# cc-ai/climategan

Hardware: AMD Instinct MI355X
Metric: 640x640 images/sec (G+D step): per-domain sample slots per second of the joint Masker+Painter training step (update_G + update_D), global batch 32 per domain (higher is better)
Workload: dtype bf16

## Files before the change

### climategan_amd/_lib.py

```python
import ctypes as C
import os
from pathlib import Path

_HERE = Path(__file__).resolve().parent
LIB_PATH = Path(os.environ["CGAN_LIB"]).resolve() if os.environ.get("CGAN_LIB") else _HERE / "libcgan_hip.so"

CGAN_F16, CGAN_BF16, CGAN_F32 = 0, 1, 2
ACT_NONE, ACT_RELU, ACT_LRELU, ACT_TANH, ACT_SIGMOID = 0, 1, 2, 3, 4
PAD_ZERO, PAD_REFLECT = 0, 1
ABI_VERSION = 1


class ConvDesc(C.Structure):
    _fields_ = [
        ("dtype", C.c_int32), ("n", C.c_int32), ("h_in", C.c_int32), ("w_in", C.c_int32),
        ("c_in", C.c_int32), ("c_out", C.c_int32),
        ("kh", C.c_int32), ("kw", C.c_int32), ("stride", C.c_int32), ("pad", C.c_int32), ("dilation", C.c_int32),
        ("pad_mode", C.c_int32), ("h_out", C.c_int32), ("w_out", C.c_int32), ("in_upsample", C.c_int32),
        ("act", C.c_int32), ("act_slope", C.c_float), ("has_bias", C.c_int32), ("has_residual", C.c_int32),
        ("residual_upsample", C.c_int32),
    ]


class NormStatsDesc(C.Structure):
# ... 121 lines not shown
    "cgan_spade_packed_weight_bytes": (C.c_size_t, [C.POINTER(SpadeDesc)]),
    "cgan_spade_pack_weights": (C.c_int, [_P, _P, _P, _P, _P, _P, _P, C.POINTER(SpadeDesc), _P]),
    "cgan_spade_fused_fwd": (C.c_int, [_P, _P, _P, _P, _P, _P, C.POINTER(SpadeDesc), _P]),
    "cgan_spade_fused_fwd_train": (C.c_int, [_P, _P, _P, _P, _P, _P, _P, C.POINTER(SpadeDesc), _P]),
    "cgan_spectral_norm_workspace_bytes": (C.c_size_t, [C.c_int32, C.c_int32]),
    "cgan_spectral_norm_power_iter": (C.c_int, [_P, _P, _P, _P, C.c_int32, C.c_int32, _P, C.c_size_t, _P]),
    "cgan_spectral_norm_power_iter_batched": (C.c_int, [_P, C.c_int32, C.c_int32, C.c_int32, _P]),
    "cgan_extra_adam_multi_tensor": (C.c_int, [_P, C.c_int32, C.c_int64, C.c_int32, C.c_int32, C.c_int32, C.c_double,
                                               C.c_double, C.c_double, C.c_double, C.c_double, _P]),
    "cgan_grads_nonfinite_check_multi_tensor": (C.c_int, [_P, C.c_int32, C.c_int64, C.c_double, C.c_int32, _P, _P]),
    "cgan_adam_multi_tensor": (C.c_int, [_P, C.c_int32, C.c_int64] + [C.c_double] * 6 + [_P, _P]),
    "cgan_rmsprop_multi_tensor": (C.c_int, [_P, C.c_int32, C.c_int64] + [C.c_double] * 5 + [_P, _P]),
    "cgan_amp_optim_finish": (C.c_int, [_P, C.c_int32, _P, _P]),
    "cgan_nchw_to_nhwc": (C.c_int, [_P, _P, _P, C.c_int32, C.c_int32, C.c_int32, C.c_int32, C.c_int32, C.c_int32, _P]),
    "cgan_nhwc_to_nchw": (C.c_int, [_P, _P, _P, _P, C.c_int32, C.c_int32, C.c_int32, C.c_int32, C.c_int32, C.c_int32, _P]),
    "cgan_resize_nearest_nhwc": (C.c_int, [_P, _P, C.c_int32, C.c_int32, C.c_int32, C.c_int32, C.c_int32, C.c_int32,
                                           C.c_int32, C.c_int32, C.c_int32, _P]),
    "cgan_avgpool3x3s2_nhwc": (C.c_int, [_P, _P, C.c_int32, C.c_int32, C.c_int32, C.c_int32, C.c_int32, _P]),
    "cgan_maxpool3x3s2_nhwc": (C.c_int, [_P, _P, C.c_int32, C.c_int32, C.c_int32, C.c_int32, C.c_int32, _P]),
    "cgan_resize_bilinear_nhwc": (C.c_int, [_P, _P, C.c_int32, C.c_int32, C.c_int32, C.c_int32, C.c_int32, C.c_int32,
                                            C.c_int32, C.c_int32, _P]),
    "cgan_resize_bicubic_nhwc": (C.c_int, [_P, _P, C.c_int32, C.c_int32, C.c_int32, C.c_int32, C.c_int32, C.c_int32,
                                           C.c_int32, _P]),
    "cgan_sumpool2x2_nhwc": (C.c_int, [_P, _P, C.c_int32, C.c_int32, C.c_int32, C.c_int32, C.c_int32, _P]),
    "cgan_reflect_pad_bwd_nhwc": (C.c_int, [_P, _P, C.c_int32, C.c_int32, C.c_int32, C.c_int32, C.c_int32, C.c_int32, _P]),
    "cgan_copy_channels_nhwc": (C.c_int, [_P, _P, C.c_int64, C.c_int32, C.c_int32, C.c_int32, C.c_int32, _P]),
    "cgan_eltwise_nhwc": (C.c_int, [_P, _P, _P, C.c_int32, C.c_int32, C.c_int64, _P]),
    "cgan_fold_bn": (C.c_int, [_P, _P, _P, _P, _P, _P, C.c_float, _P, _P, C.c_int32, C.c_int64, _P]),
    "cgan_act_bwd": (C.c_int, [_P, _P, _P, C.c_int32, C.c_int32, C.c_float, C.c_int64, _P]),
    "cgan_instnorm_act_bwd_workspace_bytes": (C.c_size_t, [C.POINTER(NormStatsDesc)]),
    "cgan_instnorm_act_bwd": (C.c_int, [_P, _P, _P, _P, C.POINTER(NormStatsDesc), C.c_int32, C.c_float, _P, C.c_size_t,
                                        _P]),
    "cgan_spade_bwd_prepare": (C.c_int, [_P, _P, _P, _P, _P, _P, _P, _P, _P, C.POINTER(SpadeDesc), _P]),
    "cgan_spade_hidden_bwd_workspace_bytes": (C.c_size_t, [C.POINTER(SpadeDesc)]),
    "cgan_spade_hidden_bwd": (C.c_int, [_P, _P, _P, _P, _P, _P, _P, _P, C.c_size_t, C.POINTER(SpadeDesc), _P]),
    "cgan_batchnorm_train_stats": (C.c_int, [_P, _P, _P, C.c_float, _P, _P, _P, _P, _P, _P, _P, C.POINTER(NormStatsDesc), _P,
                                             C.c_size_t, _P]),
    "cgan_batchnorm_train_stats_from_partials": (C.c_int, [_P, C.c_int32, _P, _P, C.c_float, _P, _P, _P, _P, _P, _P, _P,
                                                           C.POINTER(NormStatsDesc), _P]),
    "cgan_conv2d_stats_chunk_pixels": (C.c_int32, [C.POINTER(ConvDesc)]),
    "cgan_conv2d_nhwc_fwd_stats": (C.c_int, [_P, _P, _P, _P, _P, C.c_size_t, C.POINTER(ConvDesc), _P]),
    "cgan_bn_train_prepare": (C.c_int, [_P, _P, _P, _P, C.c_float, C.c_float, C.c_int64, _P, _P, _P, _P, _P, C.c_int32, _P]),
    "cgan_batchnorm_act_bwd_workspace_bytes": (C.c_size_t, [C.c_int32]),
    "cgan_batchnorm_act_bwd": (C.c_int, [_P, _P, _P, _P, _P, _P, _P, _P, _P, _P, _P, _P, C.c_int32, C.c_int64, C.c_int32,
                                         C.c_int32, C.c_float, _P, C.c_size_t, _P]),
    "cgan_batchnorm_act_bwd_grouped": (C.c_int, [_P, _P, _P, _P, _P, _P, _P, _P, _P, _P, _P, _P, C.c_int32, C.c_int64,
                                                 C.c_int32, C.c_int32, C.c_int32, C.c_float, _P, C.c_size_t, _P]),
    "cgan_bce_logits_nhwc": (C.c_int, [_P, C.c_int32, C.c_int64, C.c_int32, C.c_float, C.c_float, _P, _P, _P]),
    "cgan_hinge_nhwc": (C.c_int, [_P, C.c_int32, C.c_int64, C.c_int32, C.c_int32, C.c_int32, C.c_float, _P, _P, _P]),
    "cgan_l1_nhwc": (C.c_int, [_P, _P, C.c_int32, C.c_int64, C.c_float, _P, _P, _P]),
    "cgan_mse_const_nhwc": (C.c_int, [_P, C.c_int32, C.c_int64, C.c_int32, C.c_float, C.c_float, _P, _P, _P]),
    "cgan_painter_aux_losses": (C.c_int, [_P, _P, _P, C.c_int32, C.c_int32, C.c_int32, C.c_int32, C.c_float, C.c_float,
                                          C.c_float, C.c_float, _P, _P, _P]),
    "cgan_resize_bicubic_bwd_nhwc": (C.c_int, [_P, _P, C.c_int32, C.c_int32, C.c_int32, C.c_int32, C.c_int32, C.c_int32,
                                               C.c_int32, _P]),
    "cgan_spectral_norm_bwd": (C.c_int, [_P, _P, _P, _P, _P, C.c_int32, C.c_int32, _P, _P]),
    "cgan_painter_heads_fwd": (C.c_int, [_P, _P, _P, _P, _P, C.c_int32, C.c_int32, C.c_int32, C.c_int32, _P]),
    "cgan_painter_heads_bwd": (C.c_int, [_P, _P, _P, _P, C.c_int32, C.c_int32, C.c_int32, C.c_int32, _P]),
    "cgan_diffaug_fwd": (C.c_int, [_P, _P, _P, _P, C.c_int32, C.c_int32, C.c_int32, C.c_int32, C.c_int32, C.c_int32,
                                   C.c_int32, _P, _P]),
    "cgan_diffaug_bwd": (C.c_int, [_P, _P, _P, _P, C.c_int32, C.c_int32, C.c_int32, C.c_int32, C.c_int32, C.c_int32,
                                   C.c_int32, _P, _P]),
    "cgan_painter_heads_diffaug_fwd": (C.c_int, [_P, _P, _P, _P, _P, _P, _P, C.c_int32, C.c_int32, C.c_int32, C.c_int32,
                                                 C.c_int32, C.c_int32, C.c_int32, _P, _P]),
    "cgan_painter_heads_diffaug_bwd": (C.c_int, [_P, _P, _P, _P, _P, _P, C.c_int32, C.c_int32, C.c_int32, C.c_int32,
                                                 C.c_int32, C.c_int32, C.c_int32, _P, _P]),
# ... 149 lines not shown
```

### climategan_amd/autograd.py

```python
import ctypes as C

import os

import torch

from . import ops


GRAD_SCALE = 1.0


def set_grad_scale(s: float):
    global GRAD_SCALE
    GRAD_SCALE = float(s)


BN_GROUPS = 1


class bn_groups:

    def __init__(self, groups: int):
        self.groups = int(groups)

# ... 197 lines not shown
                                       pad_mode=cfg.get("pad_mode", ops.PAD_ZERO), add=add, prepacked=ctx.dgrad,
                                       relu_out=relu_out).t
        dw = db = None
        if ctx.needs_input_grad[1] or (ctx.has_bias and ctx.needs_input_grad[2]):
            dw, db = ops.conv2d_bwd_weight(
                ops.NHWC(x_t, cfg["c_in"]), dy, tuple(weight.shape), stride=cfg["stride"], pad=cfg["pad"],
                dilation=cfg["dilation"], want_bias=ctx.has_bias, pad_mode=cfg.get("pad_mode", ops.PAD_ZERO))
        return dx_t, dw, db, None, None


class InstNormActFn(torch.autograd.Function):

    @staticmethod
    def forward(ctx, x_t, c, eps, act, slope):
        x = ops.NHWC(x_t, c)
        mean, rstd = ops.instnorm_stats(x, eps=eps)
        out = ops.norm_act_apply(x, mean, rstd, act=act, slope=slope)
        ctx.c, ctx.act, ctx.slope = c, act, slope
        ctx.save_for_backward(out.t, rstd)
        return out.t

    @staticmethod
    def backward(ctx, dy_t):
        out_t, rstd = ctx.saved_tensors
        dx = ops.instnorm_act_bwd(ops.NHWC(out_t, ctx.c), ops.NHWC(dy_t.contiguous(), ctx.c), rstd, act=ctx.act,
                                  slope=ctx.slope)
        return dx.t, None, None, None, None


_SPADE_REMAT_GAMMA = os.environ.get("CGAN_SPADE_REMAT_GAMMA") == "1"


_SPADE_FUSED_BWD = os.environ.get("CGAN_SPADE_FUSED_BWD", "1") != "0"


class SpadeFn(torch.autograd.Function):

    @staticmethod
    def forward(ctx, x_t, cond_t, mean, rstd, w_sh, b_sh, w_g, b_g, w_b, b_b, packed, cfg):
        x = ops.NHWC(x_t, cfg["c"])
        cond = ops.NHWC(cond_t, cfg["cond_c"])
        gamma_t = None
        if _SPADE_REMAT_GAMMA or not any(ctx.needs_input_grad):
            y = ops.spade_fused(x, mean, rstd, cond, packed, act=cfg["act"], slope=cfg["slope"],
                                x_upsample=cfg["x_upsample"])
        else:
            y, gamma = ops.spade_fused(x, mean, rstd, cond, packed, act=cfg["act"], slope=cfg["slope"],
                                       x_upsample=cfg["x_upsample"], want_gamma=True)
            gamma_t = gamma.t
        ctx.cfg = cfg
        ctx.save_for_backward(x_t, cond_t, mean, rstd, y.t, w_sh, b_sh, w_g, b_g, w_b, b_b, gamma_t)
        return y.t

    @staticmethod
    def backward(ctx, dy_t):
        cfg = ctx.cfg
        x_t, cond_t, mean, rstd, y_t, w_sh, b_sh, w_g, b_g, w_b, b_b, gamma_t = ctx.saved_tensors
        c, dt = cfg["c"], y_t.dtype
        x, y = ops.NHWC(x_t, c), ops.NHWC(y_t, c)
        dy = ops.NHWC(dy_t.contiguous(), c)
        h, w = y.h, y.w
        seg = ops.resize_nearest(ops.NHWC(cond_t, cfg["cond_c"]), (h, w), cs_out=ops.cs8(cfg["cond_c"]))
        pw_sh = ops.pack_conv_weight(w_sh, b_sh, dt)
        actv = ops.conv2d(seg, pw_sh, pad=1, act=ops.ACT_RELU)
        gamma = ops.NHWC(gamma_t, c) if gamma_t is not None else ops.conv2d(actv, ops.pack_conv_weight(w_g, b_g, dt), pad=1)
        dgb, xhat, dxhat = ops.spade_bwd_prepare(dy, y, x, mean, rstd, gamma, act=cfg["act"], slope=cfg["slope"],
                                                 x_upsample=cfg["x_upsample"])
        del gamma
        w_gb = torch.cat([w_g.detach(), w_b.detach()], dim=0)
        want_gb, want_sh = any(ctx.needs_input_grad[6:10]), any(ctx.needs_input_grad[4:6])
        dw_gb = db_gb = dw_sh = db_sh = None
        if want_gb:
            dw_gb, db_gb = ops.conv2d_bwd_weight(actv, dgb, tuple(w_gb.shape), pad=1)
        fused = (_SPADE_FUSED_BWD and want_sh and not ctx.needs_input_grad[1] and cfg["cond_c"] <= 4 and h * w >= 6400
                 and w_sh.shape[0] == 128 and dgb.t.nbytes < ops.ABI_MAX_BYTES and seg.t.nbytes < ops.ABI_MAX_BYTES)
        d_pre = None
        if fused:
            dw_sh, db_sh = ops.spade_hidden_bwd(dgb, w_gb, seg, pw_sh, c)
        elif want_sh or ctx.needs_input_grad[1]:
            d_pre = ops.conv2d_bwd_data(dgb, w_gb, (actv.n, h, w), pad=1, relu_out=actv)
        del dgb, actv
        if want_sh and not fused:
            dw_sh, db_sh = ops.conv2d_bwd_weight(seg, d_pre, tuple(w_sh.shape), pad=1)
        dcond_t = None
        if ctx.needs_input_grad[1]:
            d_seg = ops.conv2d_bwd_data(d_pre, w_sh.detach(), (seg.n, h, w), pad=1)
            dcond_t = ops.resize_nearest_bwd(d_seg, (cond_t.shape[1], cond_t.shape[2]), cond_t.shape[3]).t
        del d_pre
        if cfg.get("batch_stats"):
            nn_, hh, ww, cs = xhat.t.shape
            dx = ops.instnorm_act_bwd(ops.NHWC(xhat.t.view(1, nn_ * hh * ww, 1, cs), c),
                                      ops.NHWC(dxhat.t.view(1, nn_ * hh * ww, 1, cs), c), rstd[0:1].contiguous(),
                                      act=ops.ACT_NONE)
            dx = ops.NHWC(dx.t.view(nn_, hh, ww, cs), c)
        else:
            dx = ops.instnorm_act_bwd(xhat, dxhat, rstd, act=ops.ACT_NONE)
        if cfg["x_upsample"]:
            dx = ops.sumpool2x2(dx)
        dx_t = dx.t if ctx.needs_input_grad[0] else None
        if not want_gb:
            return (dx_t, dcond_t, None, None, dw_sh, db_sh, None, None, None, None, None, None)
        return (dx_t, dcond_t, None, None, dw_sh, db_sh, dw_gb[:c].contiguous(), db_gb[:c].contiguous(),
                dw_gb[c:].contiguous(), db_gb[c:].contiguous(), None, None)


class MakeMCondFn(torch.autograd.Function):

    @staticmethod
    def forward(ctx, d_t, s_t, x, s_c):
        ctx.s_c, ctx.with_x = s_c, x is not None
        ctx.save_for_backward(d_t, s_t)
        return ops.make_m_cond(ops.NHWC(d_t, 1), ops.NHWC(s_t, s_c), x).t

    @staticmethod
    def backward(ctx, dcond_t):
        d_t, s_t = ctx.saved_tensors
        cond_c = 1 + ctx.s_c + (3 if ctx.with_x else 0)
        dd, ds = ops.make_m_cond_bwd(ops.NHWC(dcond_t.contiguous(), cond_c), ops.NHWC(d_t, 1), ops.NHWC(s_t, ctx.s_c),
                                     ctx.with_x)
        return dd.t, ds.t, None, None


class PainterHeadsFn(torch.autograd.Function):

    @staticmethod
    def forward(ctx, fake_t, x, m, want_d, want_vgg):
        d_in, v_in = ops.painter_heads(ops.NHWC(fake_t, 3), x, m, fake_t.dtype, want_d, want_vgg)
        ctx.save_for_backward(m)
        ctx.want = (want_d, want_vgg)
        empty = fake_t.new_empty(0)
# ... 547 lines not shown
```

### climategan_amd/csrc/train_ops.hip

```cpp
#include "cgan_common.h"

namespace {

__host__ __device__ inline int grid_for_n(long total) {
  long g = (total + 255) / 256;
  return (int)(g < 1 ? 1 : (g > 8192 ? 8192 : g));
}

__device__ __forceinline__ float act_grad_from_out(float out, int act, float slope) {
  switch (act) {
    case CGAN_ACT_RELU: return out > 0.f ? 1.f : 0.f;
    case CGAN_ACT_LRELU: return out > 0.f ? 1.f : slope;
    case CGAN_ACT_TANH: return 1.f - out * out;
    case CGAN_ACT_SIGMOID: return out * (1.f - out);
    default: return 1.f;
  }
}

template <typename T>
__global__ void act_bwd_kernel(const uint16_t* __restrict__ out, const uint16_t* dy, uint16_t* dx, int act, float slope,
                               long groups) {
  for (long i = (long)blockIdx.x * blockDim.x + threadIdx.x; i < groups; i += (long)gridDim.x * blockDim.x) {
    const u32x4 o = CGAN_LD_STREAM(reinterpret_cast<const u32x4*>(out) + i);
    const u32x4 g = CGAN_LD_STREAM(reinterpret_cast<const u32x4*>(dy) + i);
// ... 206 lines not shown
        const float xh = live ? (xv[hh] - mean[(long)n * cs + ch]) * rstd[(long)n * cs + ch] : 0.f;
        rxh[hh] = xh;
        rdx[hh] = dz * (1.f + g2[hh]);
        rdg[hh] = dz * xh;
        dbeta[2 * e + hh] = dz;
      }
      oxh[e] = pack2<T>(rxh[0], rxh[1]);
      odx[e] = pack2<T>(rdx[0], rdx[1]);
      odg[e] = pack2<T>(rdg[0], rdg[1]);
    }
    CGAN_ST_STREAM(oxh, reinterpret_cast<u32x4*>(xhat) + i);
    CGAN_ST_STREAM(odx, reinterpret_cast<u32x4*>(dxhat) + i);
    uint16_t* row = dgb + pix * cs2;
    if (cg * 8 + 8 <= c) {
      *reinterpret_cast<u32x4*>(row + cg * 8) = odg;
    } else {
#pragma unroll
      for (int e = 0; e < 8; ++e)
        if (cg * 8 + e < c) row[cg * 8 + e] = (uint16_t)((odg[e >> 1] >> ((e & 1) * 16)) & 0xffffu);
    }
    if (cg * 8 + 8 <= c && (c & 3) == 0) {
      const u32x4 obt = {pack2<T>(dbeta[0], dbeta[1]), pack2<T>(dbeta[2], dbeta[3]), pack2<T>(dbeta[4], dbeta[5]),
                         pack2<T>(dbeta[6], dbeta[7])};
      if ((c & 7) == 0) {
        *reinterpret_cast<u32x4*>(row + c + cg * 8) = obt;
      } else {
        *reinterpret_cast<u32x2*>(row + c + cg * 8) = (u32x2){obt[0], obt[1]};
        *reinterpret_cast<u32x2*>(row + c + cg * 8 + 4) = (u32x2){obt[2], obt[3]};
      }
    } else {
#pragma unroll
      for (int e = 0; e < 8; ++e)
        if (cg * 8 + e < c) row[c + cg * 8 + e] = bits_of<T>(dbeta[e]);
    }
  }
}

__global__ void bn_train_prepare_kernel(const float* __restrict__ mean, const float* __restrict__ rstd,
                                        const float* __restrict__ gamma, const float* __restrict__ beta, float eps,
                                        float momentum, float count, float* __restrict__ running_mean,
                                        float* __restrict__ running_var, float* __restrict__ mean_out,
                                        float* __restrict__ rstd_out, long long* __restrict__ num_batches_tracked, int c,
                                        int cs) {
  const int ch = blockIdx.x * blockDim.x + threadIdx.x;
  if (ch == 0 && num_batches_tracked) *num_batches_tracked += 1;
  if (ch >= cs) return;
  float m = 0.f, r = 0.f;
  if (ch < c) {
    const float mu = mean[ch], rs = rstd[ch];
    r = rs * (gamma ? gamma[ch] : 1.f);
    m = mu - ((beta && r != 0.f) ? beta[ch] / r : 0.f);
    if (running_mean) {
      const float var_b = 1.f / (rs * rs) - eps;
      const float var_u = count > 1.f ? var_b * count / (count - 1.f) : var_b;
      running_mean[ch] = (1.f - momentum) * running_mean[ch] + momentum * mu;
      running_var[ch] = (1.f - momentum) * running_var[ch] + momentum * var_u;
    }
  }
  mean_out[ch] = m;
  rstd_out[ch] = r;
}

constexpr int BN_BWD_MAX_CHUNKS = 512;
template <int MASK>
__device__ __forceinline__ float bn_bwd_act_grad(float ov, float xv, float fm, float fr, float gneg) {
  if (MASK == 0) return 1.f;
// ... 312 lines not shown
    long blocks = (d->hw + (long)rows * 4 - 1) / ((long)rows * 4);
    const long cap = 8192 / d->n > 0 ? 8192 / d->n : 1;
    blocks = blocks < 1 ? 1 : (blocks > cap ? cap : blocks);
    DISPATCH_T(d->dtype, in_bwd_apply_kernel, dim3((unsigned)blocks, d->n), dim3(256), 0, s, (const uint16_t*)out,
               (const uint16_t*)dy, rstd, (const float*)workspace, (uint16_t*)dx, d->hw, cs, d->c, act, act_slope);
  }
  CGAN_CHECK_LAUNCH("instnorm_act_bwd");
  return CGAN_OK;
}

extern "C" int cgan_spade_bwd_prepare(const void* dy, const void* y, const void* x, const float* mean, const float* rstd,
                                      const void* gamma, void* dgb, void* xhat, void* dxhat, const CganSpadeDesc* d,
                                      void* stream) {
  CGAN_REQUIRE(d && dy && y && x && mean && rstd && gamma && dgb && xhat && dxhat, "spade_bwd_prepare: null pointer");
  CGAN_REQUIRE(d->dtype == CGAN_F16 || d->dtype == CGAN_BF16, "spade_bwd_prepare: bad dtype %d", d->dtype);
  CGAN_REQUIRE(d->n > 0 && d->h > 0 && d->w > 0 && d->c > 0, "spade_bwd_prepare: bad shape");
  CGAN_REQUIRE(d->act == CGAN_ACT_NONE || d->act == CGAN_ACT_LRELU, "spade_bwd_prepare: Unsupported activation: %d", d->act);
  if (d->x_upsample) CGAN_REQUIRE((d->h % 2) == 0 && (d->w % 2) == 0, "spade_bwd_prepare: x_upsample needs even h/w");
  const int cs = cgan_cs(d->c), cs2 = cgan_cs(2 * d->c);
  const long npix = (long)d->n * d->h * d->w;
  hipStream_t s = (hipStream_t)stream;
  if (cs2 != 2 * d->c) {
    hipError_t e = hipMemsetAsync(dgb, 0, (size_t)npix * cs2 * 2, s);
    if (e != hipSuccess) {
      cgan_set_error("spade_bwd_prepare: hipMemsetAsync failed: %s", hipGetErrorString(e));
      return CGAN_ERR_HIP;
    }
  }
  const long groups = npix * (cs / 8);
  DISPATCH_T(d->dtype, spade_bwd_prepare_kernel, dim3(grid_for_n(groups)), dim3(256), 0, s, (const uint16_t*)dy,
             (const uint16_t*)y, (const uint16_t*)x, mean, rstd, (const uint16_t*)gamma, (uint16_t*)dgb, (uint16_t*)xhat,
             (uint16_t*)dxhat, d->h, d->w, d->c, cs, cs2, d->x_upsample, d->act, d->act_slope, groups);
  CGAN_CHECK_LAUNCH("spade_bwd_prepare");
  return CGAN_OK;
}

extern "C" int cgan_bn_train_prepare(const float* batch_mean, const float* batch_rstd, const float* gamma,
                                     const float* beta, float eps, float momentum, int64_t count, float* running_mean,
                                     float* running_var, float* mean_out, float* rstd_out,
                                     int64_t* num_batches_tracked, int32_t c, void* stream) {
  CGAN_REQUIRE(batch_mean && batch_rstd && mean_out && rstd_out, "bn_train_prepare: null pointer");
  CGAN_REQUIRE((running_mean == nullptr) == (running_var == nullptr), "bn_train_prepare: running stats go together");
  CGAN_REQUIRE(c > 0 && count > 0, "bn_train_prepare: bad shape");
  const int cs = cgan_cs(c);
  hipLaunchKernelGGL(bn_train_prepare_kernel, dim3((cs + 255) / 256), dim3(256), 0, (hipStream_t)stream, batch_mean,
                     batch_rstd, gamma, beta, eps, momentum, (float)count, running_mean, running_var, mean_out, rstd_out,
                     (long long*)num_batches_tracked, c, cs);
  CGAN_CHECK_LAUNCH("bn_train_prepare");
  return CGAN_OK;
}

extern "C" size_t cgan_batchnorm_act_bwd_workspace_bytes(int32_t c) {
  return c > 0 ? (size_t)cgan_cs(c) * (3 + 2 * (size_t)BN_BWD_MAX_CHUNKS) * sizeof(float) : 0;
}

extern "C" int cgan_batchnorm_act_bwd(const void* x, const void* out, const void* dy, const float* batch_mean,
                                      const float* batch_rstd, const float* gamma, const float* fold_mean,
                                      const float* fold_rstd, void* dx, float* dgamma, float* dbeta, void* dz_out,
                                      int32_t dtype, int64_t npix, int32_t c, int32_t act, float act_slope,
                                      void* workspace, size_t workspace_bytes, void* stream) {
  return cgan_batchnorm_act_bwd_grouped(x, out, dy, batch_mean, batch_rstd, gamma, fold_mean, fold_rstd, dx, dgamma, dbeta,
                                        dz_out, dtype, npix, c, 1, act, act_slope, workspace, workspace_bytes, stream);
}

extern "C" int cgan_batchnorm_act_bwd_grouped(const void* x, const void* out, const void* dy, const float* batch_mean,
                                              const float* batch_rstd, const float* gamma, const float* fold_mean,
// ... 75 lines not shown
```

### climategan_amd/ops.py

```python
import collections
import ctypes as C
import functools
import inspect
import os
from dataclasses import dataclass
from typing import Optional, Tuple

import torch

from . import _lib
from ._lib import (ACT_LRELU, ACT_NONE, ACT_RELU, ACT_SIGMOID, ACT_TANH, CGAN_BF16, CGAN_F16, PAD_REFLECT,
                   PAD_ZERO, ConvDesc, NormStatsDesc, PackItem, SnItem, SpadeDesc)

_DT = {torch.float16: CGAN_F16, torch.bfloat16: CGAN_BF16}


def touch(*tensors) -> None:
    ts = [t for t in tensors if t is not None]
    if ts:
        torch.autograd.graph.increment_version(ts)


MAX_MAP_BYTES = 2 ** 31
ABI_MAX_BYTES = 2 ** 31
# ... 1345 lines not shown
    if x.c != pk.c or cond.c != pk.cond_c:
        raise RuntimeError("spade_fused: channel mismatch (x %d vs %d, cond %d vs %d)" % (x.c, pk.c, cond.c, pk.cond_c))
    if cond.cs != cs4(cond.c):
        raise RuntimeError("spade_fused: cond must be stored with round_up(cond_c,4) channels")
    if x.t.dtype != pk.dtype or cond.t.dtype != pk.dtype:
        raise RuntimeError("spade_fused: dtype mismatch")
    h, w = (x.h * 2, x.w * 2) if x_upsample else (x.h, x.w)
    d = _spade_desc(x.dtype_id, x.n, h, w, x.c, x_upsample, cond.h, cond.w, cond.c, act, slope)
    y = _empty((x.n, h, w, x.cs), dtype=x.t.dtype, device=x.t.device)
    lib = _lib.load()
    if want_gamma:
        gamma = _empty_like(y)
        _lib.check(lib.cgan_spade_fused_fwd_train(_ptr(x.t), _ptr(mean), _ptr(rstd), _ptr(cond.t), _ptr(pk.buf), _ptr(y),
                                                  _ptr(gamma), C.byref(d), _stream()), "cgan_spade_fused_fwd_train")
        return NHWC(y, x.c), NHWC(gamma, x.c)
    _lib.check(lib.cgan_spade_fused_fwd(_ptr(x.t), _ptr(mean), _ptr(rstd), _ptr(cond.t), _ptr(pk.buf), _ptr(y),
                                        C.byref(d), _stream()), "cgan_spade_fused_fwd")
    return NHWC(y, x.c)


@_batch_chunked("dy", "y", "x", "mean", "rstd", "gamma", out_bytes_per_sample=lambda g: g("y").h * g("y").w * cs8(2 * g("y").c) * 2)
def spade_bwd_prepare(dy: NHWC, y: NHWC, x: NHWC, mean, rstd, gamma: NHWC, act=ACT_NONE, slope=0.2, x_upsample=False):
    _need_cuda(dy.t, y.t, x.t, mean, rstd, gamma.t)
    c = y.c
    d = _spade_desc(y.dtype_id, y.n, y.h, y.w, c, x_upsample, y.h, y.w, 3, act, slope)
    dgb = _empty((y.n, y.h, y.w, cs8(2 * c)), dtype=y.t.dtype, device=y.t.device)
    xhat = _empty_like(y.t)
    dxhat = _empty_like(y.t)
    lib = _lib.load()
    _lib.check(lib.cgan_spade_bwd_prepare(_ptr(dy.t), _ptr(y.t), _ptr(x.t), _ptr(mean), _ptr(rstd), _ptr(gamma.t),
                                          _ptr(dgb), _ptr(xhat), _ptr(dxhat), C.byref(d), _stream()),
               "cgan_spade_bwd_prepare")
    return NHWC(dgb, 2 * c), NHWC(xhat, c), NHWC(dxhat, c)


@_batch_chunked("x", "mean", "rstd", "gamma", "beta")
def pair_spade_apply(x: "PairMap", mean, rstd, gamma: "PairMap", beta: "PairMap", act=ACT_NONE, slope=0.2,
                     x_upsample=False) -> "PairMap":
    _need_cuda(x.t, mean, rstd, gamma.t, beta.t)
    h, w = (x.h * 2, x.w * 2) if x_upsample else (x.h, x.w)
    if (gamma.n, gamma.h, gamma.w, gamma.c) != (x.n, h, w, x.c) or gamma.t.shape != beta.t.shape or gamma.t.dtype != x.t.dtype:
        raise RuntimeError("pair_spade_apply: gamma / beta must be pair maps of x's channels at the output extent")
    y = _empty((x.n, h, w, x.nb * x.cs), dtype=x.t.dtype, device=x.t.device)
    _lib.check(_lib.load().cgan_pair_spade_apply(_ptr(x.t), _ptr(mean), _ptr(rstd), _ptr(gamma.t), _ptr(beta.t), _ptr(y), x.dtype_id,
                                                 x.n, h, w, x.c, int(bool(x_upsample)), int(act), float(slope), _stream()),
               "cgan_pair_spade_apply")
    return PairMap(y, x.c)


def spade_hidden_bwd(dgb: NHWC, w_gb: torch.Tensor, seg: NHWC, pw_shared: PackedConv, c: int, want_bias=True):
    _need_cuda(dgb.t, w_gb, seg.t)
    n, h, w = dgb.n, dgb.h, dgb.w
    hidden = w_gb.shape[1]
    if seg.c > 4 or hidden != 128 or (seg.n, seg.h, seg.w) != (n, h, w) or dgb.c != 2 * c or w_gb.shape[0] != 2 * c:
        raise RuntimeError("spade_hidden_bwd: needs a <= 4-channel conditioning image at the map's extent and hidden width 128")
    lib = _lib.load()
    w_gb = w_gb.detach().contiguous().float()
    dconv = _conv_desc(dgb.dtype_id, n, h, w, hidden, 2 * c, 3, 3, 1, 1, 1, PAD_ZERO, has_bias=False)
    nbytes = lib.cgan_conv2d_dgrad_packed_weight_bytes(C.byref(dconv))
    if nbytes == 0:
        _lib.check(-1, "cgan_conv2d_dgrad_packed_weight_bytes")
    packed = _empty(nbytes, dtype=torch.uint8, device=w_gb.device)
    _lib.check(lib.cgan_conv2d_pack_weight_dgrad(_ptr(w_gb), _ptr(None), _ptr(packed), C.byref(dconv), _stream()),
               "cgan_conv2d_pack_weight_dgrad")
    d = _spade_desc(dgb.dtype_id, n, h, w, c, False, h, w, seg.c, ACT_NONE)
    ws = _empty(lib.cgan_spade_hidden_bwd_workspace_bytes(C.byref(d)), dtype=torch.uint8, device=dgb.t.device)
# ... 504 lines not shown
```

### include/climategan_hip.h

```cpp
#ifndef CLIMATEGAN_HIP_H
#define CLIMATEGAN_HIP_H

#include <stddef.h>
#include <stdint.h>

#ifdef __cplusplus
extern "C" {
#endif

#define CGAN_ABI_VERSION 1

typedef enum {
  CGAN_OK = 0,
  CGAN_ERR_BAD_ARG = -1,
  CGAN_ERR_UNSUPPORTED = -2,
  CGAN_ERR_WORKSPACE = -3,
  CGAN_ERR_HIP = -4
} cgan_status_t;

typedef enum { CGAN_F16 = 0, CGAN_BF16 = 1, CGAN_F32 = 2  } cgan_dtype_t;
typedef enum { CGAN_ACT_NONE = 0, CGAN_ACT_RELU = 1, CGAN_ACT_LRELU = 2, CGAN_ACT_TANH = 3, CGAN_ACT_SIGMOID = 4 } cgan_act_t;
typedef enum { CGAN_PAD_ZERO = 0, CGAN_PAD_REFLECT = 1 } cgan_pad_t;

static inline int cgan_cs(int c) { return (c + 7) & ~7; }
// ... 137 lines not shown

int cgan_nchw_to_nhwc(const float* x, const float* mask, void* y, int32_t dtype, int32_t n, int32_t c, int32_t h,
                      int32_t w, int32_t cs, void* stream);
int cgan_nhwc_to_nchw(const void* y, const float* paste_x, const float* paste_m, float* out, int32_t dtype,
                      int32_t n, int32_t c, int32_t h, int32_t w, int32_t cs, void* stream);
int cgan_resize_nearest_nhwc(const void* x, void* y, int32_t dtype, int32_t n, int32_t c, int32_t h_in, int32_t w_in,
                             int32_t cs_in, int32_t h_out, int32_t w_out, int32_t cs_out, void* stream);
int cgan_avgpool3x3s2_nhwc(const void* x, void* y, int32_t dtype, int32_t n, int32_t c, int32_t h_in, int32_t w_in,
                           void* stream);

int cgan_maxpool3x3s2_nhwc(const void* x, void* y, int32_t dtype, int32_t n, int32_t c, int32_t h_in, int32_t w_in,
                           void* stream);
int cgan_resize_bilinear_nhwc(const void* x, void* y, int32_t dtype, int32_t n, int32_t c, int32_t h_in, int32_t w_in,
                              int32_t h_out, int32_t w_out, int32_t align_corners, void* stream);
int cgan_resize_bicubic_nhwc(const void* x, void* y, int32_t dtype, int32_t n, int32_t c, int32_t h_in, int32_t w_in,
                             int32_t h_out, int32_t w_out, void* stream);
int cgan_sumpool2x2_nhwc(const void* x, void* y, int32_t dtype, int32_t n, int32_t c, int32_t h_out, int32_t w_out,
                         void* stream);
int cgan_reflect_pad_bwd_nhwc(const void* dx_padded, void* dx, int32_t dtype, int32_t n, int32_t c, int32_t h, int32_t w,
                              int32_t pad, void* stream);
int cgan_copy_channels_nhwc(const void* src, void* dst, int64_t npix, int32_t c, int32_t cs_src, int32_t cs_dst,
                            int32_t c_off, void* stream);
int cgan_eltwise_nhwc(const void* a, const void* b, void* y, int32_t dtype, int32_t op, int64_t numel, void* stream);
int cgan_fold_bn(const float* w, const float* bias, const float* gamma, const float* beta, const float* mean,
                 const float* var, float eps, float* w_out, float* b_out, int32_t c_out, int64_t per_out, void* stream);

int cgan_act_bwd(const void* out, const void* dy, void* dx, int32_t dtype, int32_t act, float act_slope,
                 int64_t numel, void* stream);
size_t cgan_instnorm_act_bwd_workspace_bytes(const CganNormStatsDesc* d);
int cgan_instnorm_act_bwd(const void* out, const void* dy, const float* rstd, void* dx, const CganNormStatsDesc* d,
                          int32_t act, float act_slope, void* workspace, size_t workspace_bytes, void* stream);
int cgan_spade_bwd_prepare(const void* dy, const void* y, const void* x, const float* mean, const float* rstd,
                           const void* gamma, void* dgb, void* xhat, void* dxhat, const CganSpadeDesc* d, void* stream);
size_t cgan_spade_hidden_bwd_workspace_bytes(const CganSpadeDesc* d);
int cgan_spade_hidden_bwd(const void* dgb, const void* packed_dgrad_gb, const void* cond_hw, const void* packed_w_shared,
                          const float* bias_shared_padded, float* dw_shared, float* db_shared, void* workspace,
                          size_t workspace_bytes, const CganSpadeDesc* d, void* stream);
int cgan_bn_train_prepare(const float* batch_mean, const float* batch_rstd, const float* gamma, const float* beta,
                          float eps, float momentum, int64_t count, float* running_mean, float* running_var,
                          float* mean_out, float* rstd_out, int64_t* num_batches_tracked, int32_t c, void* stream);
int cgan_batchnorm_train_stats(const void* x, const float* gamma, const float* beta, float momentum, float* running_mean,
                               float* running_var, int64_t* num_batches_tracked, float* batch_mean, float* batch_rstd,
                               float* mean_out, float* rstd_out, const CganNormStatsDesc* d, void* workspace,
                               size_t workspace_bytes, void* stream);
int cgan_batchnorm_train_stats_from_partials(float* partial, int32_t chunk_pixels, const float* gamma,
                                             const float* beta, float momentum, float* running_mean, float* running_var,
                                             int64_t* num_batches_tracked, float* batch_mean, float* batch_rstd,
                                             float* mean_out, float* rstd_out, const CganNormStatsDesc* d, void* stream);
size_t cgan_batchnorm_act_bwd_workspace_bytes(int32_t c);
int cgan_batchnorm_act_bwd(const void* x, const void* out, const void* dy, const float* batch_mean,
                           const float* batch_rstd, const float* gamma, const float* fold_mean, const float* fold_rstd,
                           void* dx, float* dgamma, float* dbeta, void* dz_out, int32_t dtype, int64_t npix, int32_t c,
                           int32_t act, float act_slope, void* workspace, size_t workspace_bytes, void* stream);
int cgan_batchnorm_act_bwd_grouped(const void* x, const void* out, const void* dy, const float* batch_mean,
                                   const float* batch_rstd, const float* gamma, const float* fold_mean,
                                   const float* fold_rstd, void* dx, float* dgamma, float* dbeta, void* dz_out,
                                   int32_t dtype, int64_t npix_total, int32_t c, int32_t groups, int32_t act,
                                   float act_slope, void* workspace, size_t workspace_bytes, void* stream);
int cgan_bce_logits_nhwc(const void* x, int32_t dtype, int64_t npix, int32_t c, float target, float weight,
                         float* loss_accum, void* dx, void* stream);
int cgan_hinge_nhwc(const void* x, int32_t dtype, int64_t npix, int32_t c, int32_t target_is_real,
                    int32_t for_discriminator, float weight, float* loss_accum, void* dx, void* stream);
int cgan_mse_const_nhwc(const void* x, int32_t dtype, int64_t npix, int32_t c, float target, float weight, float* loss_accum,
                        void* dx, void* stream);
int cgan_painter_aux_losses(const void* fake_nhwc, const float* x_nchw, const float* m_nchw, int32_t dtype, int32_t n,
                            int32_t h, int32_t w, float w_tv_h, float w_tv_w, float w_context, float w_reconstruction,
// ... 260 lines not shown
```

Measured before the change: 57.36.

## Fuse SPADE backward prepare, instnorm backward and upsample sumpool into chained kernels

Adds a spade_bwd_chain path that computes dgamma/dbeta and dxhat while accumulating the instance-norm backward partial sums in the same pass, then finishes with a dx kernel that also folds in the 2x2 sumpool for the upsampled case. This removes the materialised xhat tensor, the separate instnorm_act_bwd stats pass and the sumpool kernel in the SPADE backward. It is on by default for non-batch-stats SPADE layers and adds bf16 rounding points chosen to match the old path's intermediate precision.

```diff
diff --git a/climategan_amd/_lib.py b/climategan_amd/_lib.py
--- a/climategan_amd/_lib.py
+++ b/climategan_amd/_lib.py
@@ -177,6 +177,8 @@
     "cgan_instnorm_act_bwd": (C.c_int, [_P, _P, _P, _P, C.POINTER(NormStatsDesc), C.c_int32, C.c_float, _P, C.c_size_t,
                                         _P]),
     "cgan_spade_bwd_prepare": (C.c_int, [_P, _P, _P, _P, _P, _P, _P, _P, _P, C.POINTER(SpadeDesc), _P]),
+    "cgan_spade_bwd_chain_workspace_bytes": (C.c_size_t, [C.POINTER(SpadeDesc)]),
+    "cgan_spade_bwd_chain": (C.c_int, [_P, _P, _P, _P, _P, _P, _P, _P, _P, C.POINTER(SpadeDesc), _P, C.c_size_t, _P]),
     "cgan_spade_hidden_bwd_workspace_bytes": (C.c_size_t, [C.POINTER(SpadeDesc)]),
     "cgan_spade_hidden_bwd": (C.c_int, [_P, _P, _P, _P, _P, _P, _P, _P, C.c_size_t, C.POINTER(SpadeDesc), _P]),
     "cgan_batchnorm_train_stats": (C.c_int, [_P, _P, _P, C.c_float, _P, _P, _P, _P, _P, _P, _P, C.POINTER(NormStatsDesc), _P,
diff --git a/climategan_amd/autograd.py b/climategan_amd/autograd.py
--- a/climategan_amd/autograd.py
+++ b/climategan_amd/autograd.py
@@ -253,6 +253,7 @@
 
 
 _SPADE_FUSED_BWD = os.environ.get("CGAN_SPADE_FUSED_BWD", "1") != "0"
+_SPADE_BWD_CHAIN = os.environ.get("CGAN_SPADE_BWD_CHAIN", "1") != "0"
 
 
 class SpadeFn(torch.autograd.Function):
@@ -285,8 +286,13 @@
         pw_sh = ops.pack_conv_weight(w_sh, b_sh, dt)
         actv = ops.conv2d(seg, pw_sh, pad=1, act=ops.ACT_RELU)
         gamma = ops.NHWC(gamma_t, c) if gamma_t is not None else ops.conv2d(actv, ops.pack_conv_weight(w_g, b_g, dt), pad=1)
-        dgb, xhat, dxhat = ops.spade_bwd_prepare(dy, y, x, mean, rstd, gamma, act=cfg["act"], slope=cfg["slope"],
-                                                 x_upsample=cfg["x_upsample"])
+        chain = _SPADE_BWD_CHAIN and not cfg.get("batch_stats")
+        if chain:
+            dgb, dx = ops.spade_bwd_chain(dy, y, x, mean, rstd, gamma, act=cfg["act"], slope=cfg["slope"],
+                                          x_upsample=cfg["x_upsample"])
+        else:
+            dgb, xhat, dxhat = ops.spade_bwd_prepare(dy, y, x, mean, rstd, gamma, act=cfg["act"], slope=cfg["slope"],
+                                                     x_upsample=cfg["x_upsample"])
         del gamma
         w_gb = torch.cat([w_g.detach(), w_b.detach()], dim=0)
         want_gb, want_sh = any(ctx.needs_input_grad[6:10]), any(ctx.needs_input_grad[4:6])
@@ -308,7 +314,9 @@
             d_seg = ops.conv2d_bwd_data(d_pre, w_sh.detach(), (seg.n, h, w), pad=1)
             dcond_t = ops.resize_nearest_bwd(d_seg, (cond_t.shape[1], cond_t.shape[2]), cond_t.shape[3]).t
         del d_pre
-        if cfg.get("batch_stats"):
+        if chain:
+            pass
+        elif cfg.get("batch_stats"):
             nn_, hh, ww, cs = xhat.t.shape
             dx = ops.instnorm_act_bwd(ops.NHWC(xhat.t.view(1, nn_ * hh * ww, 1, cs), c),
                                       ops.NHWC(dxhat.t.view(1, nn_ * hh * ww, 1, cs), c), rstd[0:1].contiguous(),
@@ -316,7 +324,7 @@
             dx = ops.NHWC(dx.t.view(nn_, hh, ww, cs), c)
         else:
             dx = ops.instnorm_act_bwd(xhat, dxhat, rstd, act=ops.ACT_NONE)
-        if cfg["x_upsample"]:
+        if cfg["x_upsample"] and not chain:
             dx = ops.sumpool2x2(dx)
         dx_t = dx.t if ctx.needs_input_grad[0] else None
         if not want_gb:
diff --git a/climategan_amd/csrc/train_ops.hip b/climategan_amd/csrc/train_ops.hip
--- a/climategan_amd/csrc/train_ops.hip
+++ b/climategan_amd/csrc/train_ops.hip
@@ -262,6 +262,223 @@
 #pragma unroll
       for (int e = 0; e < 8; ++e)
         if (cg * 8 + e < c) row[c + cg * 8 + e] = bits_of<T>(dbeta[e]);
+    }
+  }
+}
+
+template <typename T>
+__device__ __forceinline__ void round2(float& a, float& b) {
+  unpack2<T>(pack2<T>(a, b), a, b);
+}
+
+template <typename T, bool UPS>
+__global__ __launch_bounds__(256) void spade_bwd_split_kernel(
+    const uint16_t* __restrict__ dy, const uint16_t* __restrict__ y, const uint16_t* __restrict__ x,
+    const float* __restrict__ mean, const float* __restrict__ rstd, const uint16_t* __restrict__ gamma,
+    uint16_t* __restrict__ dgb, uint16_t* __restrict__ dxhat, float* __restrict__ partial, int h, int w, int c, int cs,
+    int cs2, int ppb, int act, float slope) {
+  extern __shared__ __attribute__((aligned(16))) float sm[];
+  const int hw = h * w;
+  const int cg_total = cs / 8;
+  const int cgb = cg_total < 256 ? cg_total : 256;
+  const int PL = 256 / cgb;
+  const int n = blockIdx.z, cg0 = blockIdx.y * cgb;
+  const int p0 = blockIdx.x * ppb, p1 = min(hw, p0 + ppb);
+  const int t = threadIdx.x, cgl = t % cgb, pl = t / cgb;
+  const int cg = cg0 + cgl;
+  float s1[8], s2[8];
+#pragma unroll
+  for (int e = 0; e < 8; ++e) s1[e] = s2[e] = 0.f;
+  if (pl < PL && cg < cg_total) {
+    const int nlive = c - cg * 8;
+    const float neg = act == CGAN_ACT_LRELU ? slope : 1.f;
+    float mu[8], rs[8];
+#pragma unroll
+    for (int e = 0; e < 8; ++e) {
+      mu[e] = mean[(size_t)n * cs + cg * 8 + e];
+      rs[e] = rstd[(size_t)n * cs + cg * 8 + e];
+    }
+    const size_t pix0 = (size_t)n * hw;
+    const size_t xn = (size_t)n * (h >> 1) * (w >> 1);
+    int oy = 0, ox = 0;
+    if (UPS) {
+      oy = (p0 + pl) / w;
+      ox = (p0 + pl) - oy * w;
+    }
+#pragma unroll 2
+    for (int p = p0 + pl; p < p1; p += PL) {
+      const size_t pix = pix0 + p;
+      const size_t off = pix * cs + cg * 8;
+      size_t xoff = off;
+      if (UPS) {
+        xoff = (xn + (size_t)(oy >> 1) * (w >> 1) + (ox >> 1)) * cs + cg * 8;
+        ox += PL;
+        while (ox >= w) {
+          ox -= w;
+          ++oy;
+        }
+      }
+      const u32x4 vdy = *reinterpret_cast<const u32x4*>(dy + off);
+      const u32x4 vy = *reinterpret_cast<const u32x4*>(y + off);
+      const u32x4 vg = *reinterpret_cast<const u32x4*>(gamma + off);
+      const u32x4 vx = *reinterpret_cast<const u32x4*>(x + xoff);
+      u32x4 odx, odg;
+      float dbeta[8];
+#pragma unroll
+      for (int e = 0; e < 4; ++e) {
+        float a[2], b[2], g2[2], xv[2], rxh[2], rdx[2], rdg[2];
+        unpack2<T>(vdy[e], a[0], a[1]);
+        unpack2<T>(vy[e], b[0], b[1]);
+        unpack2<T>(vg[e], g2[0], g2[1]);
+        unpack2<T>(vx[e], xv[0], xv[1]);
+#pragma unroll
+        for (int hh = 0; hh < 2; ++hh) {
+          const int k = 2 * e + hh;
+          const bool live = k < nlive;
+          const float dz = live ? a[hh] * (b[hh] > 0.f ? 1.f : neg) : 0.f;
+          const float xh = live ? (xv[hh] - mu[k]) * rs[k] : 0.f;
+          rxh[hh] = xh;
+          rdx[hh] = dz * (1.f + g2[hh]);
+          rdg[hh] = dz * xh;
+          dbeta[k] = dz;
+        }
+        odx[e] = pack2<T>(rdx[0], rdx[1]);
+        odg[e] = pack2<T>(rdg[0], rdg[1]);
+        unpack2<T>(odx[e], rdx[0], rdx[1]);
+        round2<T>(rxh[0], rxh[1]);
+#pragma unroll
+        for (int hh = 0; hh < 2; ++hh) {
+          s1[2 * e + hh] += rdx[hh];
+          s2[2 * e + hh] = __builtin_fmaf(rdx[hh], rxh[hh], s2[2 * e + hh]);
+        }
+      }
+      CGAN_ST_STREAM(odx, reinterpret_cast<u32x4*>(dxhat + off));
+      uint16_t* row = dgb + pix * cs2;
+      if (nlive >= 8) {
+        *reinterpret_cast<u32x4*>(row + cg * 8) = odg;
+      } else {
+#pragma unroll
+        for (int e = 0; e < 8; ++e)
+          if (e < nlive) row[cg * 8 + e] = (uint16_t)((odg[e >> 1] >> ((e & 1) * 16)) & 0xffffu);
+      }
+      if (nlive >= 8 && (c & 3) == 0) {
+        const u32x4 obt = {pack2<T>(dbeta[0], dbeta[1]), pack2<T>(dbeta[2], dbeta[3]), pack2<T>(dbeta[4], dbeta[5]),
+                           pack2<T>(dbeta[6], dbeta[7])};
+        if ((c & 7) == 0) {
+          *reinterpret_cast<u32x4*>(row + c + cg * 8) = obt;
+        } else {
+          *reinterpret_cast<u32x2*>(row + c + cg * 8) = (u32x2){obt[0], obt[1]};
+          *reinterpret_cast<u32x2*>(row + c + cg * 8 + 4) = (u32x2){obt[2], obt[3]};
+        }
+      } else {
+#pragma unroll
+        for (int e = 0; e < 8; ++e)
+          if (e < nlive) row[c + cg * 8 + e] = bits_of<T>(dbeta[e]);
+      }
+    }
+  }
+  if (pl < PL) {
+#pragma unroll
+    for (int e = 0; e < 8; ++e) {
+      sm[((pl * cgb + cgl) * 8 + e) * 2] = s1[e];
+      sm[((pl * cgb + cgl) * 8 + e) * 2 + 1] = s2[e];
+    }
+  }
+  __syncthreads();
+  for (int ch = t; ch < cgb * 8; ch += 256) {
+    if (cg0 * 8 + ch >= cs) continue;
+    float a = 0.f, b = 0.f;
+    for (int l = 0; l < PL; ++l) {
+      a += sm[((l * cgb) * 8 + ch) * 2];
+      b += sm[((l * cgb) * 8 + ch) * 2 + 1];
+    }
+    float* o = partial + (((size_t)n * gridDim.x + blockIdx.x) * cs + cg0 * 8 + ch) * 2;
+    o[0] = a;
+    o[1] = b;
+  }
+}
+
+template <typename T, bool UPS>
+__global__ __launch_bounds__(256) void spade_bwd_dx_kernel(const uint16_t* __restrict__ x,
+                                                           const uint16_t* __restrict__ dxhat,
+                                                           const float* __restrict__ mean, const float* __restrict__ rstd,
+                                                           const float* __restrict__ sums, uint16_t* __restrict__ dx, int h,
+                                                           int w, int cs, int c) {
+  const int cg_total = cs / 8;
+  const int tpp = cg_total < 256 ? cg_total : 256;
+  const int rows = 256 / tpp;
+  const int cgl = threadIdx.x % tpp, prow = threadIdx.x / tpp;
+  if (prow >= rows) return;
+  const int n = blockIdx.y;
+  const int hw = h * w;
+  const float inv_hw = 1.f / (float)hw;
+  const int np = UPS ? hw >> 2 : hw;
+  const int wl = w >> 1;
+  dxhat += (size_t)n * hw * cs;
+  x += (size_t)n * np * cs;
+  dx += (size_t)n * np * cs;
+  for (int cg = cgl; cg < cg_total; cg += tpp) {
+    const int nlive = c - cg * 8;
+    float rs[8], m1[8], m2[8], mu[8];
+#pragma unroll
+    for (int e = 0; e < 8; ++e) {
+      const int ch = cg * 8 + e;
+      const float* sp = sums + ((size_t)n * cs + ch) * 2;
+      rs[e] = rstd[(size_t)n * cs + ch];
+      mu[e] = mean[(size_t)n * cs + ch];
+      m1[e] = sp[0] * inv_hw;
+      m2[e] = sp[1] * inv_hw;
+    }
+#pragma unroll 2
+    for (int p = blockIdx.x * rows + prow; p < np; p += gridDim.x * rows) {
+      const size_t off = (size_t)p * cs + cg * 8;
+      const u32x4 vx = CGAN_LD_STREAM(reinterpret_cast<const u32x4*>(x + off));
+      u32x4 vd[UPS ? 4 : 1];
+      if constexpr (UPS) {
+        const int qy = (int)((unsigned)p / (unsigned)wl), qx = p - qy * wl;
+        const uint16_t* b0 = dxhat + ((size_t)(2 * qy) * w + 2 * qx) * cs + cg * 8;
+        const uint16_t* b1 = b0 + (size_t)w * cs;
+        vd[0] = CGAN_LD_STREAM(reinterpret_cast<const u32x4*>(b0));
+        vd[1] = CGAN_LD_STREAM(reinterpret_cast<const u32x4*>(b0 + cs));
+        vd[2] = CGAN_LD_STREAM(reinterpret_cast<const u32x4*>(b1));
+        vd[3] = CGAN_LD_STREAM(reinterpret_cast<const u32x4*>(b1 + cs));
+      } else {
+        vd[0] = CGAN_LD_STREAM(reinterpret_cast<const u32x4*>(dxhat + off));
+      }
+      u32x4 r;
+#pragma unroll
+      for (int e = 0; e < 4; ++e) {
+        float xv[2], yv[2];
+        unpack2<T>(vx[e], xv[0], xv[1]);
+#pragma unroll
+        for (int hh = 0; hh < 2; ++hh) {
+          const int k = 2 * e + hh;
+          yv[hh] = k < nlive ? (xv[hh] - mu[k]) * rs[k] : 0.f;
+        }
+        round2<T>(yv[0], yv[1]);
+        float acc[2] = {0.f, 0.f};
+#pragma unroll
+        for (int j = 0; j < (UPS ? 4 : 1); ++j) {
+          float dz[2], res[2];
+          unpack2<T>(vd[j][e], dz[0], dz[1]);
+#pragma unroll
+          for (int hh = 0; hh < 2; ++hh) {
+            const int k = 2 * e + hh;
+            const float v = rs[k] * __builtin_fmaf(-yv[hh], m2[k], dz[hh] - m1[k]);
+            res[hh] = k < nlive ? v : 0.f;
+          }
+          if (UPS) {
+            round2<T>(res[0], res[1]);
+            acc[0] += res[0];
+            acc[1] += res[1];
+          } else {
+            acc[0] = res[0];
+            acc[1] = res[1];
+          }
+        }
+        r[e] = pack2<T>(acc[0], acc[1]);
+      }
+      CGAN_ST_STREAM(r, reinterpret_cast<u32x4*>(dx + off));
     }
   }
 }
@@ -640,6 +857,77 @@
              (const uint16_t*)y, (const uint16_t*)x, mean, rstd, (const uint16_t*)gamma, (uint16_t*)dgb, (uint16_t*)xhat,
              (uint16_t*)dxhat, d->h, d->w, d->c, cs, cs2, d->x_upsample, d->act, d->act_slope, groups);
   CGAN_CHECK_LAUNCH("spade_bwd_prepare");
+  return CGAN_OK;
+}
+
+#define DISPATCH_T_UPS(dtype, ups, KERNEL, ...)                                    \
+  do {                                                                             \
+    if (ups) DISPATCH_T2(dtype, KERNEL, true, __VA_ARGS__);                        \
+    else DISPATCH_T2(dtype, KERNEL, false, __VA_ARGS__);                           \
+  } while (0)
+
+static CganNormStatsDesc spade_bwd_chain_norm_desc(const CganSpadeDesc* d) {
+  CganNormStatsDesc nd;
+  nd.dtype = d->dtype;
+  nd.n = d->n;
+  nd.hw = d->h * d->w;
+  nd.c = d->c;
+  nd.eps = 0.f;
+  return nd;
+}
+
+extern "C" size_t cgan_spade_bwd_chain_workspace_bytes(const CganSpadeDesc* d) {
+  if (!d || d->n <= 0 || d->c <= 0 || d->h <= 0 || d->w <= 0 || (long)d->h * d->w > 0x7fffffffL) return 0;
+  const CganNormStatsDesc nd = spade_bwd_chain_norm_desc(d);
+  return cgan_instnorm_act_bwd_workspace_bytes(&nd);
+}
+
+extern "C" int cgan_spade_bwd_chain(const void* dy, const void* y, const void* x, const float* mean, const float* rstd,
+                                    const void* gamma, void* dgb, void* dxhat, void* dx, const CganSpadeDesc* d,
+                                    void* workspace, size_t workspace_bytes, void* stream) {
+  CGAN_REQUIRE(d && dy && y && x && mean && rstd && gamma && dgb && dxhat && dx && workspace,
+               "spade_bwd_chain: null pointer");
+  CGAN_REQUIRE(d->dtype == CGAN_F16 || d->dtype == CGAN_BF16, "spade_bwd_chain: bad dtype %d", d->dtype);
+  CGAN_REQUIRE(d->n > 0 && d->h > 0 && d->w > 0 && d->c > 0, "spade_bwd_chain: bad shape");
+  CGAN_REQUIRE(d->act == CGAN_ACT_NONE || d->act == CGAN_ACT_LRELU, "spade_bwd_chain: Unsupported activation: %d", d->act);
+  if (d->x_upsample) CGAN_REQUIRE((d->h % 2) == 0 && (d->w % 2) == 0, "spade_bwd_chain: x_upsample needs even h/w");
+  const int cs = cgan_cs(d->c), cs2 = cgan_cs(2 * d->c);
+  const long npix = (long)d->n * d->h * d->w;
+  CGAN_REQUIRE((double)npix * cs2 * 2 < 2147483648.0,
+               "spade_bwd_chain: a %d x %d x %d x %d map reaches 2 GiB; call it on batch slices", d->n, d->h, d->w, cs2);
+  CGAN_REQUIRE(workspace_bytes >= cgan_spade_bwd_chain_workspace_bytes(d), "spade_bwd_chain: workspace too small");
+  hipStream_t s = (hipStream_t)stream;
+  if (cs2 != 2 * d->c) {
+    hipError_t e = hipMemsetAsync(dgb, 0, (size_t)npix * cs2 * 2, s);
+    if (e != hipSuccess) {
+      cgan_set_error("spade_bwd_chain: hipMemsetAsync failed: %s", hipGetErrorString(e));
+      return CGAN_ERR_HIP;
+    }
+  }
+  const CganNormStatsDesc nd = spade_bwd_chain_norm_desc(d);
+  const int cg_total = cs / 8;
+  int cgb, PL, ppb, chunks;
+  in_bwd_plan(&nd, cgb, PL, ppb, chunks);
+  float* sums = (float*)workspace;
+  float* partial = sums + (size_t)d->n * cs * 2;
+  const size_t smem = (size_t)PL * cgb * 8 * 2 * sizeof(float);
+  DISPATCH_T_UPS(d->dtype, d->x_upsample, spade_bwd_split_kernel, dim3(chunks, ceil_div(cg_total, cgb), d->n), dim3(256),
+                 smem, s, (const uint16_t*)dy, (const uint16_t*)y, (const uint16_t*)x, mean, rstd, (const uint16_t*)gamma,
+                 (uint16_t*)dgb, (uint16_t*)dxhat, partial, d->h, d->w, d->c, cs, cs2, ppb, d->act, d->act_slope);
+  hipLaunchKernelGGL(in_bwd_finalize_kernel, dim3(d->n * cs / 8), dim3(256), 0, s, (const float*)partial, sums, d->n, cs,
+                     chunks);
+  {
+    const int tpp = cg_total < 256 ? cg_total : 256, rows = 256 / tpp;
+    const long np = d->x_upsample ? nd.hw / 4 : nd.hw;
+    const long per = d->x_upsample ? 1 : 4;
+    long blocks = (np + rows * per - 1) / (rows * per);
+    const long cap = 8192 / d->n > 0 ? 8192 / d->n : 1;
+    blocks = blocks < 1 ? 1 : (blocks > cap ? cap : blocks);
+    DISPATCH_T_UPS(d->dtype, d->x_upsample, spade_bwd_dx_kernel, dim3((unsigned)blocks, d->n), dim3(256), 0, s,
+                   (const uint16_t*)x, (const uint16_t*)dxhat, mean, rstd, (const float*)sums, (uint16_t*)dx, d->h, d->w, cs,
+                   d->c);
+  }
+  CGAN_CHECK_LAUNCH("spade_bwd_chain");
   return CGAN_OK;
 }
 
diff --git a/climategan_amd/ops.py b/climategan_amd/ops.py
--- a/climategan_amd/ops.py
+++ b/climategan_amd/ops.py
@@ -1401,6 +1401,32 @@
                                           _ptr(dgb), _ptr(xhat), _ptr(dxhat), C.byref(d), _stream()),
                "cgan_spade_bwd_prepare")
     return NHWC(dgb, 2 * c), NHWC(xhat, c), NHWC(dxhat, c)
+
+
+@_batch_chunked("dy", "y", "x", "mean", "rstd", "gamma", out_bytes_per_sample=lambda g: g("y").h * g("y").w * cs8(2 * g("y").c) * 2)
+def spade_bwd_chain(dy: NHWC, y: NHWC, x: NHWC, mean, rstd, gamma: NHWC, act=ACT_NONE, slope=0.2, x_upsample=False):
+    _need_cuda(dy.t, y.t, x.t, mean, rstd, gamma.t)
+    _need_cs8("spade_bwd_chain", dy, y, x, gamma)
+    c = y.c
+    xh, xw = (y.h // 2, y.w // 2) if x_upsample else (y.h, y.w)
+    if (x_upsample and (y.h % 2 or y.w % 2)) or tuple(x.t.shape) != (y.n, xh, xw, y.cs) or dy.t.shape != y.t.shape \
+            or gamma.t.shape != y.t.shape or x.c != c or tuple(mean.shape) != (y.n, y.cs) or tuple(rstd.shape) != (y.n, y.cs):
+        raise RuntimeError("spade_bwd_chain: dy, y and gamma share one shape, x has it (halved under x_upsample: even "
+                           "extents), mean / rstd are [N, Cs]")
+    for t in (dy.t, y.t, x.t, gamma.t, mean, rstd):
+        if not t.is_contiguous():
+            raise RuntimeError("spade_bwd_chain: contiguous tensors expected")
+    d = _spade_desc(y.dtype_id, y.n, y.h, y.w, c, x_upsample, y.h, y.w, 3, act, slope)
+    lib = _lib.load()
+    dgb = _empty((y.n, y.h, y.w, cs8(2 * c)), dtype=y.t.dtype, device=y.t.device)
+    dx = _empty_like(x.t)
+    dxhat = torch.empty_like(y.t)
+    nbytes = lib.cgan_spade_bwd_chain_workspace_bytes(C.byref(d))
+    ws = _empty(nbytes, dtype=torch.uint8, device=y.t.device)
+    _lib.check(lib.cgan_spade_bwd_chain(_ptr(dy.t), _ptr(y.t), _ptr(x.t), _ptr(mean), _ptr(rstd), _ptr(gamma.t), _ptr(dgb),
+                                        _ptr(dxhat), _ptr(dx), C.byref(d), _ptr(ws), nbytes, _stream()),
+               "cgan_spade_bwd_chain")
+    return NHWC(dgb, 2 * c), NHWC(dx, c)
 
 
 @_batch_chunked("x", "mean", "rstd", "gamma", "beta")
diff --git a/include/climategan_hip.h b/include/climategan_hip.h
--- a/include/climategan_hip.h
+++ b/include/climategan_hip.h
@@ -193,6 +193,10 @@
                           int32_t act, float act_slope, void* workspace, size_t workspace_bytes, void* stream);
 int cgan_spade_bwd_prepare(const void* dy, const void* y, const void* x, const float* mean, const float* rstd,
                            const void* gamma, void* dgb, void* xhat, void* dxhat, const CganSpadeDesc* d, void* stream);
+size_t cgan_spade_bwd_chain_workspace_bytes(const CganSpadeDesc* d);
+int cgan_spade_bwd_chain(const void* dy, const void* y, const void* x, const float* mean, const float* rstd,
+                         const void* gamma, void* dgb, void* dxhat, void* dx, const CganSpadeDesc* d, void* workspace,
+                         size_t workspace_bytes, void* stream);
 size_t cgan_spade_hidden_bwd_workspace_bytes(const CganSpadeDesc* d);
 int cgan_spade_hidden_bwd(const void* dgb, const void* packed_dgrad_gb, const void* cond_hw, const void* packed_w_shared,
                           const float* bias_shared_padded, float* dw_shared, float* db_shared, void* workspace,
```

Result: no change. 57.79 (median of 2 runs) (+0.8%).
